# mcdiarmid/waveforms

Measured on AMD Instinct MI355X. Metric: SOQPSK-TG Msym/s mod+Viterbi-detect @8sps, higher is better.
Workload: dtype f64; 1 GPU; SOQPSK-TG 1e+07 symbols @8 sps, modulate + AWGN + PT matched filter + 4-state Viterbi detect (BASELINE configs[1]); waveform=soqpsk, sps=8, prbs=PN23, noise=Philox4x32-10 + Box-Muller (device), fuse=175, streams=1, detector_warmup_rows=16, detector_form=lanes (one chunk per lane), parallelism=independent trial blocks x1

## Files before the change

waveforms_amd/csrc/wf_common.h:

```cpp
#pragma once
#include <hip/hip_runtime.h>
#include <stdint.h>

#include <atomic>
#include <map>
#include <mutex>
#include <vector>
#include <string>

#include "../../include/wfhip.h"

#define WF_WAVE 64

void wf_set_error(const char *fmt, ...);

#define WF_HIP(call)                                                                     \
    do {                                                                                 \
        hipError_t e_ = (call);                                                          \
        if (e_ != hipSuccess) {                                                          \
            wf_set_error("%s failed: %s (%s:%d)", #call, hipGetErrorString(e_), __FILE__, \
                         __LINE__);                                                      \
            return WF_ERR_HIP;                                                           \
        }                                                                                \
    } while (0)

#define WF_REQUIRE(cond, ...)          \
    do {                               \
        if (!(cond)) {                 \
            wf_set_error(__VA_ARGS__); \
            return WF_ERR_VALUE;       \
        }                              \
    } while (0)

#define WF_LAUNCH_CHECK() WF_HIP(hipGetLastError())

enum { WF_FAULT_SCAN_TIMEOUT = 1u, WF_FAULT_LIVE_TABLE = 2u };

struct wf_lfsr_tables {
    uint64_t host[64][64];
    uint64_t *dev = nullptr;
    uint64_t f_even = 0, f_odd = 0, f_m2 = 0, f_m1 = 0;
    bool f_ready = false;
};

struct wf_ctx {
    int device = 0;
    int cus = 256;
    int64_t opt[WF_OPT_COUNT] = {0};
    uint64_t *d_scan = nullptr;
    size_t scan_words = 0;
    unsigned *d_fault = nullptr;
    unsigned *h_fault = nullptr;
    uint8_t *d_tables = nullptr;
    uint8_t h_tables_cache[2048] = {0};
    int tables_cached = 0;
    hipEvent_t tables_event = nullptr;
    hipStream_t tables_stream = nullptr;
    bool tables_pending = false;
    uint64_t *d_fsm_scratch = nullptr;
    size_t fsm_scratch_words = 0;
    int *h_small = nullptr;
    int *d_small = nullptr;
    std::map<uint64_t, wf_lfsr_tables *> lfsr;
    double *d_mod_scratch = nullptr;
    size_t mod_scratch_words = 0;
    double *d_vit_edge = nullptr;
    size_t vit_edge_words = 0;
    unsigned long long *d_vit_unmerged = nullptr;
    hipEvent_t *events = nullptr;
    void *pipe_stream = nullptr;
    void *pipe_stream2 = nullptr;
    void *pipe_pro = nullptr, *pipe_main = nullptr;
    hipEvent_t pipe_pro_done = nullptr;
    hipEvent_t pipe_back_go = nullptr;
    bool pipe_back_go_valid = false;
    bool pipe_front_recorded = false;
    bool pipe_front_on_main = false;
    hipEvent_t pipe_front = nullptr, pipe_done[2] = {nullptr, nullptr};
    bool pipe_done_valid[2] = {false, false};
    int pipe_set = 0;
    std::map<uint64_t, uint32_t> promises;
    std::mutex promises_lock;
    double *h_iter = nullptr;
    double *d_iter = nullptr;
    void *h_mailbox = nullptr;
    void *d_mailbox = nullptr;
    void *iter_stream = nullptr;
    const void *iter_last_state = nullptr;
    std::atomic_flag iter_lock = ATOMIC_FLAG_INIT;
    bool iter_closing = false;
};

static inline hipStream_t wf_stream(void *s) { return reinterpret_cast<hipStream_t>(s); }

int wf_ctx_reserve_scan(wf_ctx *ctx, size_t words);
int wf_ctx_reserve_fsm(wf_ctx *ctx, size_t words);
int wf_ctx_reserve_mod(wf_ctx *ctx, size_t words);
int wf_iter_server_stop(wf_ctx *ctx);
int wf_ctx_reserve_vit(wf_ctx *ctx, size_t words);

struct lfsr_emit_args;
int wf_lfsr_generate_dyn(wf_ctx *ctx, int degree, uint64_t mask, uint64_t state, uint64_t skip,
                         const uint64_t *d_dyn_skip, uint8_t *d_bits, int64_t n, uint64_t *h_state_out, void *stream,
                         const struct lfsr_emit_args *emit = nullptr);
int wf_lfsr_generate_map(wf_ctx *ctx, int degree, uint64_t mask, uint64_t state, uint64_t skip, uint8_t *d_bits, int64_t nbits,
                         int map_kind, int8_t *d_symbols, void *stream);
int wf_soqpsk_prbs_encode(wf_ctx *ctx, int degree, uint64_t mask, uint64_t state, uint64_t skip, const uint8_t *h_next,
                          const int8_t *h_out, uint8_t *d_bits, int64_t n, int8_t *d_symbols, void *stream, void *mid_event = nullptr);
int wf_awgn_mf_bank_dyn(wf_ctx *ctx, const double *d_signal_ri, int64_t nsamp, double rot_re, double rot_im,
                        double sigma, uint64_t seed, uint64_t stream_id, uint64_t first_index,
                        const uint64_t *d_dyn_index, const double *d_taps_ri, int nfilt, int ntaps, int64_t first,
                        int step, int64_t ncols, double *d_out_ri, void *stream, int pack_par0 = -1);
int wf_viterbi4_detect_packed(wf_ctx *ctx, const double *d_rows4, int64_t ncalls, int differential, int warmup,
                              uint8_t *d_bits, int8_t *d_syms, double *d_state, void *stream);
int wf_cpm_modulate_window(wf_ctx *ctx, const int8_t *d_symbols, int64_t sym_origin, int64_t nloc, int64_t nsym_total,
                           const double *d_h, int nh, const double *d_pulse, int ntaps, int sps, double phi0,
                           int64_t tile_lo, int64_t ntiles, double *d_out_ri, int64_t out_origin,
                           const uint64_t *d_q_in, uint64_t *d_q_out, int64_t q_out_tile, void *stream);
struct wf_mcb_opts {
    const double *pam_factor = nullptr;
    bool cpm_paired = false;
    int runs_hint = 0;
    int scratch_slot = -1;
};
int wf_mod_chan_bank_packed(wf_ctx *ctx, const int8_t *d_symbols, int64_t nsym, const double *d_h, int nh,
                            const double *d_pulse, int ntaps, int sps, double phi0, const double *d_mf_taps, double rot_re,
                            double rot_im, double sigma, uint64_t seed, uint64_t stream_id, uint64_t first_index,
                            int64_t first, int64_t ncols, int pack_par0, double *d_rows4, void *stream, int mf_ntaps = 0,
                            const wf_mcb_opts *opts = nullptr, int stage = 3);
int wf_mod_chan_bank_window(wf_ctx *ctx, const int8_t *d_symbols, int64_t sym_origin, int64_t nloc, int64_t nsym_total,
                            const double *d_h, int nh, const double *d_pulse, int ntaps, int sps, double phi0,
                            int64_t tile_lo, int64_t ntiles, const uint64_t *d_q_in, uint64_t *d_q_out, int64_t q_out_tile,
                            const double *d_mf_taps, double rot_re, double rot_im, double sigma, uint64_t seed,
                            uint64_t stream_id, uint64_t first_index, const uint64_t *d_dyn_index, int64_t first,
                            int64_t k_lo, int64_t ncols, int pack_par0, double *d_rows4, void *stream, int cpm_nf = 0, int cpm_nh = 1,
                            int stage = 3, int mf_ntaps = 0, const wf_mcb_opts *opts = nullptr);
int wf_mod_chan_bank_applies(int64_t nsym, int nh, int ntaps, int sps, int mf_ntaps, int64_t first);
int wf_link_join_internal(wf_ctx *ctx, void *stream);
int wf_mod_chan_cpm_rows_applies(int64_t nsym, int nh, int ntaps, int sps, int nfilt, int ntm, int64_t start0);
int wf_mod_chan_cpm_rows(wf_ctx *ctx, const int8_t *d_symbols, int64_t nsym, const double *d_h, int nh, const double *d_pulse,
                         int ntaps, int sps, double phi0, const double *d_templates, int nfilt, int ntm, int64_t start0,
                         double rot_re, double rot_im, double sigma, uint64_t seed, uint64_t stream_id, int64_t ncalls,
                         double *d_rows, void *stream, const wf_mcb_opts *opts = nullptr);
int wf_mod_chan_samples_applies(int64_t nsym, int nh, int ntaps, int sps);
int wf_mod_chan_samples(wf_ctx *ctx, const int8_t *d_symbols, int64_t nsym, const double *d_h, int nh, const double *d_pulse, int ntaps,
                        int sps, double phi0, double rot_re, double rot_im, double sigma, uint64_t seed, uint64_t stream_id,
                        uint64_t first_index, double *d_out_ri, void *stream);
int wf_mod_chan_samples_window(wf_ctx *ctx, const int8_t *d_symbols, int64_t sym_origin, int64_t nloc, int64_t nsym_total, const double *d_h, int nh,
                               const double *d_pulse, int ntaps, int sps, double phi0, int64_t tile_lo, int64_t ntiles, const uint64_t *d_q_in,
                               uint64_t *d_q_out, int64_t q_out_tile, double rot_re, double rot_im, double sigma, uint64_t seed, uint64_t stream_id,
                               uint64_t first_index, double *d_out_ri, int64_t out_origin, int64_t out_hi, void *stream);
int wf_promise_verified(wf_ctx *ctx, int kind, const void *const *d_ptrs, const size_t *nbytes, int nptrs, void *stream,
                        bool (*check)(const unsigned char *const *host, const size_t *nbytes, const void *arg), const void *arg, const char *what);
int wf_fsm_encode_core(wf_ctx *ctx, const uint8_t *h_next, const int8_t *h_out, int columns, int states, int card,
                       const uint8_t *d_bits, int64_t nbits, int64_t i0, int state0, const int *d_state_in,
                       int8_t *d_symbols, int *h_state_out, int *d_state_at, int64_t at_index, void *stream);

static inline int wf_grid_for(int64_t work_items, int per_block, int max_blocks)
{
    int64_t b = (work_items + per_block - 1) / per_block;
// ... 374 lines not shown
```

waveforms_amd/csrc/wf_cpm_detect.hip:

```cpp
#include <stddef.h>
#include <stdlib.h>
#include <string.h>

#include <type_traits>

#include "wf_cpm_detect.h"
#include "wf_link.h"

#define CPM_THREADS 256
#define CPM_WAVES (CPM_THREADS / WF_WAVE)
#define CPM_GROUPS 4
#define CPM_TB 4
#define CPM_DEFAULT_WARMUP 256
#define CPM_XS 68

struct cpm_tables {
    uint8_t dest[3][16][4];
    uint16_t info[3][16][4];
};

struct cpm_vit_params {
    int M, lgM, p, nh, K0, K1, Lp, NC, D, S, NF;
    int CH, W;
    int64_t ncalls, nchunks;
// ... 1052 lines not shown
extern "C" int wf_cpm_link_run(wf_ctx *ctx, const wf_cpm_link_config *cfg, void *d_workspace, int64_t workspace_bytes,
                               int64_t *d_counts, int64_t *h_compared, void *stream)
{
    WF_REQUIRE(ctx && cfg && d_workspace && d_counts, "wf_cpm_link_run: NULL argument");
    cpm_link_layout L;
    WF_REQUIRE(cpm_make_layout(cfg, L), "wf_cpm_link_run: bad configuration");
    WF_REQUIRE((reinterpret_cast<uintptr_t>(d_workspace) & 255) == 0, "wf_cpm_link_run: workspace must be 256-byte aligned");
    WF_REQUIRE((int64_t)L.total <= workspace_bytes, "wf_cpm_link_run: workspace too small (%lld < %lld)",
               (long long)workspace_bytes, (long long)L.total);
    WF_REQUIRE(cfg->d_h && cfg->d_pulse && cfg->d_templates && cfg->d_rot_cs, "wf_cpm_link_run: NULL table pointer");
    char *w = static_cast<char *>(d_workspace);
    const bool piped = (cfg->fuse & 32) != 0 && L.ncalls > 0 && !cpm_link_samples_form_quad(cfg, L);
    int rc;
    if (piped) {
        const int64_t set_bytes = round_up((int64_t)L.total, 256);
        if ((rc = link_pipe_open(ctx, "wf_cpm_link_run", set_bytes, workspace_bytes, true)) || (rc = link_pipe_select(ctx, set_bytes, w, stream))) return rc;
    } else if ((rc = wf_link_join_internal(ctx, stream))) {
        return rc;
    }
    uint8_t *bits = reinterpret_cast<uint8_t *>(w + L.off_bits);
    int8_t *syms = reinterpret_cast<int8_t *>(w + L.off_syms);
    double *sig = reinterpret_cast<double *>(w + L.off_sig);
    double *rows = reinterpret_cast<double *>(w + L.off_rows);
    uint8_t *dec = reinterpret_cast<uint8_t *>(w + L.off_dec);
    hipEvent_t *ev;
    if ((rc = link_stage_events(ctx, "wf_cpm_link_run", cfg->event_slot, ev))) return rc;
    if ((rc = mark(ev, 0, stream))) return rc;
    rc = (cfg->fuse & 16) ? 1 : wf_lfsr_generate_map(ctx, cfg->degree, cfg->mask, cfg->state, cfg->skip, bits, L.nbits, cfg->mapper_kind, syms, stream);
    if (rc < 0) return rc;
    if (rc == 1) {
        if ((rc = wf_lfsr_generate(ctx, cfg->degree, cfg->mask, cfg->state, cfg->skip, bits, L.nbits, nullptr, stream))) return rc;
        if ((rc = mark(ev, 1, stream))) return rc;
        if ((rc = wf_symbol_map(ctx, cfg->mapper_kind, bits, L.nbits, 0, 0, 0, syms, stream))) return rc;
    } else {
        if ((rc = mark(ev, 1, stream))) return rc;
    }
    if ((rc = mark(ev, 2, stream))) return rc;
    bool fused_all = false, samples_form = false;
    const bool samples_quad = cpm_link_samples_form_quad(cfg, L);
    if (cpm_link_samples_form(ctx, cfg, L)) {
        if (!samples_quad && (rc = cpm_check_paired(ctx, cfg, L.nfilt, L.ntm, stream))) return rc;
        rc = wf_mod_chan_samples(ctx, syms, cfg->nsym, cfg->d_h, cfg->det.nh, cfg->d_pulse, cfg->ntaps, cfg->sps, M_PI / 4, cos(-M_PI / 4), sin(-M_PI / 4),
                                 cfg->sigma, cfg->seed, cfg->stream_id, 0, sig, stream);
        if (rc < 0) return rc;
        samples_form = fused_all = rc == 0;
    }
    if (!fused_all && (cfg->fuse & 8) && (cfg->fuse & 2) && L.ncalls > 0) {
        wf_mcb_opts mo;
        mo.runs_hint = piped ? (L.nfilt == 4 ? 16 : 8) : 0;
        mo.cpm_paired = (cfg->fuse & 64) != 0;
        if (mo.cpm_paired && (rc = cpm_check_paired(ctx, cfg, L.nfilt, L.ntm, stream))) return rc;
        rc = wf_mod_chan_cpm_rows(ctx, syms, cfg->nsym, cfg->d_h, cfg->det.nh, cfg->d_pulse, cfg->ntaps, cfg->sps, M_PI / 4, cfg->d_templates,
                                  L.nfilt, L.ntm, L.start0, cos(-M_PI / 4), sin(-M_PI / 4), cfg->sigma, cfg->seed, cfg->stream_id, L.ncalls,
                                  rows, stream, &mo);
        if (rc < 0) return rc;
        fused_all = rc == 0;
    }
    if (!fused_all) {
        rc = wf_cpm_modulate_c128(ctx, syms, cfg->nsym, cfg->d_h, cfg->det.nh, cfg->d_pulse, cfg->ntaps, cfg->sps, M_PI / 4, sig, stream);
        if (rc < 0) return rc;
        WF_REQUIRE(rc == 0, "wf_cpm_link_run: burst / pulse outside the fused modulator (%lld symbols, %d taps)",
                   (long long)cfg->nsym, cfg->ntaps);
    }
    if ((rc = mark(ev, 3, stream)) || (rc = mark(ev, 4, stream))) return rc;
    if (fused_all) {
        if ((rc = mark(ev, 5, stream))) return rc;
    } else if (cfg->fuse & 2) {
        if ((rc = mark(ev, 5, stream))) return rc;
        if ((rc = wf_cpm_awgn_mf_rows_c128(ctx, sig, L.npts, cos(-M_PI / 4), sin(-M_PI / 4), cfg->sigma, cfg->seed, cfg->stream_id, 0,
                                           cfg->d_templates, cfg->det.nh, L.nfilt, L.ntm, L.start0, cfg->sps, L.ncalls, rows, stream))) return rc;
    } else {
        if ((rc = wf_awgn_c128(ctx, sig, L.npts, cos(-M_PI / 4), sin(-M_PI / 4), cfg->sigma, cfg->seed, cfg->stream_id, 0, sig, stream))) return rc;
        if ((rc = mark(ev, 5, stream))) return rc;
        if ((rc = wf_cpm_mf_rows_c128(ctx, sig, L.npts, cfg->d_templates, cfg->det.nh, L.nfilt, L.ntm, L.start0, cfg->sps, L.ncalls,
                                      rows, stream))) return rc;
    }
    void *back = stream;
    const bool two_back = piped && !wf_cpm_quad_applies(&cfg->det) && !wf_cpm_wide_applies(&cfg->det);
    const int edge_slot = two_back ? ctx->pipe_set : -1;
    if (piped) {
        back = two_back && ctx->pipe_set ? ctx->pipe_stream2 : ctx->pipe_stream;
        WF_HIP(hipEventRecord(ctx->pipe_front, wf_stream(stream)));
        WF_HIP(hipStreamWaitEvent(wf_stream(back), ctx->pipe_front, 0));
    }
    if ((rc = mark(ev, 6, back))) return rc;
    if (samples_form && samples_quad) {
        const cpm_mf_source mf{cfg->d_templates, L.npts, 0, L.start0};
        if ((rc = wf_cpm_viterbi_detect_in(ctx, &cfg->det, cfg->d_rot_cs, sig, L.ncalls, cfg->warmup, dec, nullptr, back, 0, 0, piped, &mf, -1))) return rc;
    } else if (samples_form) {
        const cpm_mf_source mf{cfg->d_templates, L.npts - L.start0, 0};
        if ((rc = wf_cpm_viterbi_detect_in(ctx, &cfg->det, cfg->d_rot_cs, sig + 2 * L.start0, L.ncalls, cfg->warmup, dec, nullptr, back,
                                           (int64_t)L.off_sig + 16 * L.start0, (int64_t)(L.total - L.off_sig) - L.npts * 16, piped, &mf, edge_slot)))
            return rc;
    } else if ((rc = wf_cpm_viterbi_detect_in(ctx, &cfg->det, cfg->d_rot_cs, rows, L.ncalls, cfg->warmup, dec, nullptr, back, (int64_t)L.off_rows,
                                              (int64_t)(L.total - L.off_rows) - L.ncalls * L.nfilt * 16, piped, nullptr, edge_slot)))
        return rc;
    if ((rc = mark(ev, 7, back))) return rc;
    const int64_t skip = cfg->skip_head > 0 ? cfg->skip_head : 0;
    int64_t m = L.ncalls - cfg->det.D + 1 - skip;
    if (m < 0) m = 0;
    if (m > 0)
        if ((rc = wf_cpm_count_errors(ctx, dec + skip + cfg->det.D - 1, syms + skip, cfg->det.M, m, d_counts, back))) return rc;
    if ((rc = mark(ev, 8, back))) return rc;
    if (piped && (rc = link_pipe_close(ctx, back))) return rc;
    if (h_compared) *h_compared = m;
    return WF_OK;
}

struct cpm_stream_layout : link_chunk_window {
    int64_t N, B, tile_len, spt, ntiles_total, halo, ncalls_total, m_total;
    size_t off_bits, off_syms, off_rows, off_dec, total;
    cpm_link_layout L;
    bool ok;
};

static cpm_stream_layout cpm_make_stream_layout(const wf_cpm_link_config *cfg, int64_t B, int64_t c)
{
    cpm_stream_layout S{};
    if (!cpm_make_layout(cfg, S.L) || B <= 0 || c < 0) return S;
    S.N = cfg->nsym; S.B = B;
    S.ok = wf_mod_tile_geometry(cfg->sps, cfg->ntaps, cfg->nsym, &S.tile_len, &S.spt, &S.ntiles_total) == 0;
    if (!S.ok || S.spt <= 0) { S.ok = false; return S; }
    S.halo = round_up(S.spt + 48 + cfg->det.D, 16);
    S.ncalls_total = S.L.ncalls;
    const int64_t skip = cfg->skip_head > 0 ? cfg->skip_head : 0;
    S.m_total = S.ncalls_total - cfg->det.D + 1 - skip;
    if (S.m_total < 0) S.m_total = 0;
    S.ok = B % S.spt == 0 && B % 128 == 0 && B >= 4 * S.halo &&
           ((cfg->fuse & 8) && (cfg->fuse & 2) &&
            wf_mod_chan_cpm_rows_applies(cfg->nsym, cfg->det.nh, cfg->ntaps, cfg->sps, S.L.nfilt, S.L.ntm, S.L.start0));
    static_cast<link_chunk_window &>(S) = link_chunk_window_of(B, c, S.halo, S.N, S.ncalls_total, S.spt, S.ntiles_total);
    size_t o = 0;
    const int64_t win = B + 2 * S.halo + 32;
    S.off_bits = o; o += (size_t)round_up(win * S.L.bps, 256);
    S.off_syms = o; o += (size_t)round_up(win, 256);
    S.off_rows = o; o += (size_t)round_up(B * S.L.nfilt * 16, 256);
    S.off_dec = o;  o += (size_t)round_up(B + 16, 256);
    S.total = o;
    return S;
}

extern "C" int64_t wf_cpm_link_stream_workspace_bytes(const wf_cpm_link_config *cfg, int64_t chunk_symbols)
{
    const cpm_stream_layout S = cpm_make_stream_layout(cfg, chunk_symbols, 0);
    return S.ok ? (int64_t)S.total : -1;
}

extern "C" int wf_cpm_link_stream_layout(const wf_cpm_link_config *cfg, int64_t chunk_symbols, int64_t chunk_index, int64_t *info8)
{
    if (!info8) return WF_ERR_VALUE;
    const cpm_stream_layout S = cpm_make_stream_layout(cfg, chunk_symbols, chunk_index);
    if (!S.ok) return WF_ERR_VALUE;
    info8[0] = S.ncols; info8[1] = S.k_lo; info8[2] = (int64_t)S.off_dec; info8[3] = (int64_t)S.off_syms;
    info8[4] = S.ws; info8[5] = S.ncalls_total; info8[6] = S.spt; info8[7] = (int64_t)S.off_rows;
    return WF_OK;
}

extern "C" int wf_cpm_link_stream_chunk(wf_ctx *ctx, const wf_cpm_link_config *cfg, int64_t chunk_symbols, int64_t chunk_index,
                                        void *d_state, void *d_workspace, int64_t workspace_bytes, int64_t *d_counts,
                                        int64_t *h_compared, void *stream)
{
    return wf_cpm_link_stream_chunk_phase(ctx, cfg, chunk_symbols, chunk_index, d_state, d_workspace, workspace_bytes, d_counts, h_compared, 7, stream);
}

extern "C" int wf_cpm_link_stream_chunk_phase(wf_ctx *ctx, const wf_cpm_link_config *cfg, int64_t chunk_symbols, int64_t chunk_index,
                                              void *d_state, void *d_workspace, int64_t workspace_bytes, int64_t *d_counts,
// ... 74 lines not shown
```

waveforms_amd/csrc/wf_ctx.hip:

```cpp
#include <stdarg.h>
#include <stdio.h>

#include "wf_common.h"

static thread_local char g_err[512] = "";

void wf_set_error(const char *fmt, ...)
{
    va_list ap;
    va_start(ap, fmt);
    vsnprintf(g_err, sizeof(g_err), fmt, ap);
    va_end(ap);
}

extern "C" const char *wf_version(void) { return "waveforms-amd 0.1.0 (gfx950)"; }
extern "C" const char *wf_last_error_string(void) { return g_err; }

extern "C" int wf_ctx_create(int device, wf_ctx **out)
{
    WF_REQUIRE(out != nullptr, "wf_ctx_create: out is NULL");
    int ndev = 0;
    WF_HIP(hipGetDeviceCount(&ndev));
    WF_REQUIRE(device >= 0 && device < ndev, "wf_ctx_create: device %d of %d", device, ndev);
    WF_HIP(hipSetDevice(device));
    wf_ctx *c = new wf_ctx();
    c->device = device;
    (void)hipDeviceGetAttribute(&c->cus, hipDeviceAttributeMultiprocessorCount, device);
    if (c->cus < 1) c->cus = 256;
    c->opt[WF_OPT_PIPE_RESERVE_CUS] = -1;
    WF_HIP(hipMalloc(&c->d_fault, 64));
    WF_HIP(hipMemset(c->d_fault, 0, 64));
    WF_HIP(hipHostMalloc(&c->h_fault, 64, hipHostMallocDefault));
    WF_HIP(hipMalloc(&c->d_tables, 4096));
    WF_HIP(hipMalloc(&c->d_vit_unmerged, 4 * sizeof(unsigned long long)));
    WF_HIP(hipMemset(c->d_vit_unmerged, 0, 4 * sizeof(unsigned long long)));
    WF_HIP(hipMalloc(&c->d_small, 256));
    WF_HIP(hipHostMalloc(&c->h_small, 256, hipHostMallocDefault));
    *out = c;
    int rc = wf_ctx_reserve_scan(c, 1 << 16);
    if (rc) return rc;
    return wf_ctx_reserve_fsm(c, 1 << 16);
}

extern "C" int wf_ctx_destroy(wf_ctx *c)
{
    if (!c) return WF_OK;
    (void)hipSetDevice(c->device);
    (void)wf_iter_server_stop(c);
    (void)hipDeviceSynchronize();
    for (auto &kv : c->lfsr) {
        if (kv.second->dev) (void)hipFree(kv.second->dev);
        delete kv.second;
    }
    if (c->events) {
        for (int k = 0; k < WF_LINK_EVENT_SLOTS * (WF_LINK_STAGES + 1); ++k) (void)hipEventDestroy(c->events[k]);
        delete[] c->events;
    }
    if (c->pipe_front) (void)hipEventDestroy(c->pipe_front);
    for (int k = 0; k < 2; ++k)
        if (c->pipe_done[k]) (void)hipEventDestroy(c->pipe_done[k]);
    if (c->pipe_stream) (void)hipStreamDestroy(static_cast<hipStream_t>(c->pipe_stream));
    if (c->pipe_stream2) (void)hipStreamDestroy(static_cast<hipStream_t>(c->pipe_stream2));
    if (c->pipe_pro) (void)hipStreamDestroy(static_cast<hipStream_t>(c->pipe_pro));
    if (c->pipe_main) (void)hipStreamDestroy(static_cast<hipStream_t>(c->pipe_main));
    if (c->pipe_pro_done) (void)hipEventDestroy(c->pipe_pro_done);
    if (c->pipe_back_go) (void)hipEventDestroy(c->pipe_back_go);
    if (c->d_scan) (void)hipFree(c->d_scan);
    if (c->d_fsm_scratch) (void)hipFree(c->d_fsm_scratch);
    if (c->d_mod_scratch) (void)hipFree(c->d_mod_scratch);
    if (c->d_vit_edge) (void)hipFree(c->d_vit_edge);
    if (c->d_vit_unmerged) (void)hipFree(c->d_vit_unmerged);
    if (c->d_fault) (void)hipFree(c->d_fault);
    if (c->h_fault) (void)hipHostFree(c->h_fault);
    if (c->d_tables) (void)hipFree(c->d_tables);
    if (c->tables_event) (void)hipEventDestroy(c->tables_event);
    if (c->d_small) (void)hipFree(c->d_small);
    if (c->h_small) (void)hipHostFree(c->h_small);
    if (c->h_iter) (void)hipHostFree(c->h_iter);
    if (c->iter_stream) (void)hipStreamDestroy(static_cast<hipStream_t>(c->iter_stream));
    if (c->h_mailbox) (void)hipHostFree(c->h_mailbox);
    delete c;
    return WF_OK;
}

extern "C" int wf_ctx_retire(wf_ctx *c)
{
    if (!c) return WF_OK;
    (void)hipSetDevice(c->device);
    (void)wf_iter_server_stop(c);
    if (c->pipe_stream) (void)hipStreamSynchronize(static_cast<hipStream_t>(c->pipe_stream));
    if (c->pipe_stream2) (void)hipStreamSynchronize(static_cast<hipStream_t>(c->pipe_stream2));
    if (c->pipe_pro) (void)hipStreamSynchronize(static_cast<hipStream_t>(c->pipe_pro));
    if (c->pipe_main) (void)hipStreamSynchronize(static_cast<hipStream_t>(c->pipe_main));
    return WF_OK;
}

int wf_link_join_internal(wf_ctx *c, void *stream)
{
    if (!c) return WF_OK;
    for (int k = 0; k < 2; ++k)
        if (c->pipe_done_valid[k]) WF_HIP(hipStreamWaitEvent(wf_stream(stream), c->pipe_done[k], 0));
    return WF_OK;
}

extern "C" int wf_link_join(wf_ctx *c, void *stream)
{
    WF_REQUIRE(c != nullptr, "wf_link_join: ctx is NULL");
    return wf_link_join_internal(c, stream);
}

extern "C" int wf_ctx_set_option(wf_ctx *c, int key, int64_t value)
{
    WF_REQUIRE(c != nullptr, "wf_ctx_set_option: ctx is NULL");
    WF_REQUIRE(key >= 0 && key < WF_OPT_COUNT, "wf_ctx_set_option: unknown option %d", key);
    bool ok = true;
    switch (key) {
    case WF_OPT_CPM_FORM: ok = value >= 0 && value <= 2; break;
    case WF_OPT_CPM_CHUNK_CALLS: ok = value >= 0 && value <= 8192; break;
    case WF_OPT_DET_REPAIR: case WF_OPT_DET_FINAL_VERIFY: case WF_OPT_ITERATION_SERVER: ok = value == 0 || value == 1; break;
    case WF_OPT_MCB_TAIL_PERMILLE: ok = value >= -1 && value <= 16000; break;
    case WF_OPT_PIPE_RESERVE_CUS: ok = value >= -1 && value <= 128; break;
    case WF_OPT_CPM_SAMPLES_MIN_CALLS: ok = value == 0 || (value >= 4096 && value <= ((int64_t)1 << 40)); break;
    case WF_OPT_SOFT_CHUNK_CALLS: ok = value >= 0 && value <= 8192; break;
    case WF_OPT_CPM_SOFT_CHUNK_CALLS: ok = value >= 0 && value <= 8192; break;
    }
    WF_REQUIRE(ok, "wf_ctx_set_option: value %lld outside the range of option %d", (long long)value, key);
    c->opt[key] = value;
    return WF_OK;
}

extern "C" int wf_ctx_get_option(wf_ctx *c, int key, int64_t *value)
{
    WF_REQUIRE(c != nullptr && value != nullptr, "wf_ctx_get_option: NULL argument");
    WF_REQUIRE(key >= 0 && key < WF_OPT_COUNT, "wf_ctx_get_option: unknown option %d", key);
    *value = c->opt[key];
    return WF_OK;
}

extern "C" int wf_ctx_check(wf_ctx *c, void *stream)
{
    WF_REQUIRE(c != nullptr, "wf_ctx_check: ctx is NULL");
    {
        const int rj = wf_link_join_internal(c, stream);
        if (rj) return rj;
    }
    WF_HIP(hipMemcpyAsync(c->h_fault, c->d_fault, sizeof(unsigned), hipMemcpyDeviceToHost,
                          wf_stream(stream)));
    WF_HIP(hipStreamSynchronize(wf_stream(stream)));
    unsigned f = *c->h_fault;
    if (f) {
        WF_HIP(hipMemsetAsync(c->d_fault, 0, sizeof(unsigned), wf_stream(stream)));
        wf_set_error("device fault word 0x%x (bit0 = scan hand-off timeout, bit1 = malformed live-window table)", f);
        return WF_ERR_DEVICE;
    }
    return WF_OK;
}

int wf_promise_verified(wf_ctx *c, int kind, const void *const *d_ptrs, const size_t *nbytes, int nptrs, void *stream,
                        bool (*check)(const unsigned char *const *host, const size_t *nbytes, const void *arg), const void *arg, const char *what)
{
    uint64_t key = 1469598103934665603ull;
    auto mix = [&](uint64_t v) {
        for (int b = 0; b < 8; ++b) {
            key ^= (v >> (8 * b)) & 0xFFull;
            key *= 1099511628211ull;
        }
    };
    mix((uint64_t)kind);
    for (int i = 0; i < nptrs; ++i) {
        WF_REQUIRE(d_ptrs[i] != nullptr && nbytes[i] > 0 && nbytes[i] <= (1u << 16), "%s: operand %d is NULL or larger than 64 KB", what, i);
        mix((uint64_t)reinterpret_cast<uintptr_t>(d_ptrs[i]));
        mix((uint64_t)nbytes[i]);
    }
    std::lock_guard<std::mutex> guard(c->promises_lock);
    auto it = c->promises.find(key);
    if (it != c->promises.end()) {
// ... 86 lines not shown
```

waveforms_amd/csrc/wf_link.h:

```cpp
#pragma once
#include "wf_common.h"

static inline int64_t round_up(int64_t v, int64_t a) { return (v + a - 1) / a * a; }

static inline int link_pipe_open(wf_ctx *ctx, const char *fn, int64_t set_bytes, int64_t workspace_bytes, bool second)
{
    WF_REQUIRE(2 * set_bytes <= workspace_bytes, "%s: fuse bit 5 needs two sets of intermediates (%lld bytes)", fn, (long long)(2 * set_bytes));
    WF_HIP(hipSetDevice(ctx->device));
    hipStream_t ps;
    if (!ctx->pipe_stream) {
        WF_HIP(hipStreamCreateWithFlags(&ps, hipStreamNonBlocking));
        ctx->pipe_stream = ps;
        WF_HIP(hipEventCreateWithFlags(&ctx->pipe_front, hipEventDisableTiming));
        for (int k = 0; k < 2; ++k) WF_HIP(hipEventCreateWithFlags(&ctx->pipe_done[k], hipEventDisableTiming));
    }
    if (second && !ctx->pipe_stream2) {
        WF_HIP(hipStreamCreateWithFlags(&ps, hipStreamNonBlocking));
        ctx->pipe_stream2 = ps;
    }
    return WF_OK;
}

static inline int link_pipe_select(wf_ctx *ctx, int64_t set_bytes, char *&w, void *waiter, bool on_main = false)
{
    if (ctx->pipe_front_on_main != on_main && ctx->pipe_front_recorded) WF_HIP(hipStreamWaitEvent(wf_stream(waiter), ctx->pipe_front, 0));
    ctx->pipe_front_on_main = on_main;
    ctx->pipe_front_recorded = true;
    w += (int64_t)ctx->pipe_set * set_bytes;
    if (ctx->pipe_done_valid[ctx->pipe_set]) WF_HIP(hipStreamWaitEvent(wf_stream(waiter), ctx->pipe_done[ctx->pipe_set], 0));
    return WF_OK;
}

static inline int link_pipe_close(wf_ctx *ctx, void *back)
{
    WF_HIP(hipEventRecord(ctx->pipe_done[ctx->pipe_set], wf_stream(back)));
    ctx->pipe_done_valid[ctx->pipe_set] = true;
    ctx->pipe_set ^= 1;
    return WF_OK;
}

static inline int link_stage_events(wf_ctx *ctx, const char *fn, int event_slot, hipEvent_t *&ev)
{
    ev = nullptr;
    if (event_slot < 0) return WF_OK;
    WF_REQUIRE(event_slot < WF_LINK_EVENT_SLOTS, "%s: event_slot %d", fn, event_slot);
    if (!ctx->events) {
        ctx->events = new hipEvent_t[WF_LINK_EVENT_SLOTS * (WF_LINK_STAGES + 1)];
        for (int k = 0; k < WF_LINK_EVENT_SLOTS * (WF_LINK_STAGES + 1); ++k) WF_HIP(hipEventCreate(&ctx->events[k]));
    }
    ev = ctx->events + event_slot * (WF_LINK_STAGES + 1);
    return WF_OK;
}

static inline int mark(hipEvent_t *ev, int k, void *stream)
{
    if (ev) WF_HIP(hipEventRecord(ev[k], wf_stream(stream)));
    return WF_OK;
}

struct link_chunk_window {
    int64_t k_lo, ncols, ws, nloc, tile_lo, tile_hi, ntiles, q_out_tile;
};

static inline link_chunk_window link_chunk_window_of(int64_t B, int64_t c, int64_t halo, int64_t N, int64_t ncalls_total, int64_t spt, int64_t ntiles_total)
{
    link_chunk_window W;
    W.k_lo = c * B;
    const int64_t k_hi = W.k_lo + B < ncalls_total ? W.k_lo + B : ncalls_total;
    W.ncols = k_hi > W.k_lo ? k_hi - W.k_lo : 0;
    W.ws = c * B - halo > 0 ? c * B - halo : 0;
    const int64_t we = (c + 1) * B + halo < N ? (c + 1) * B + halo : N;
    W.nloc = we > W.ws ? we - W.ws : 0;
    W.tile_lo = spt > 0 && c * B / spt - 1 > 0 ? c * B / spt - 1 : 0;
    W.tile_hi = spt > 0 ? (c + 1) * B / spt + 1 : 0;
    if (W.tile_hi > ntiles_total) W.tile_hi = ntiles_total;
    W.ntiles = W.tile_hi > W.tile_lo ? W.tile_hi - W.tile_lo : 0;
    const int64_t next_tile_lo = spt > 0 ? (c + 1) * B / spt - 1 : 0;
    W.q_out_tile = (next_tile_lo >= W.tile_lo && next_tile_lo < W.tile_hi) ? next_tile_lo - W.tile_lo : -1;
    return W;
}

struct soqpsk_trellis_tables {
    uint8_t next[2][4][2];
    int8_t outp[2][4][2];
};

static inline soqpsk_trellis_tables soqpsk_trellis(int differential)
{
    static const int8_t kOut[2][8] = {{0, 2, 0, -2, -2, 0, 2, 0}, {0, -2, 2, 0, 0, 2, -2, 0}};
    soqpsk_trellis_tables T;
    for (int c = 0; c < 2; ++c)
        for (int b = 0; b < 8; ++b) {
            const int s = b >> 1, flip = differential ? (c == 0 ? (s >> 1) : (s & 1)) : 0, inp = (b & 1) ^ flip;
            T.next[c][s][inp] = (uint8_t)(c == 0 ? (s & 1) + 2 * (b & 1) : (s & 2) + (b & 1));
            T.outp[c][s][inp] = kOut[c][b];
        }
    return T;
}
```

waveforms_amd/csrc/wf_pipeline.hip:

```cpp
#include "wf_link.h"

__global__ void time_axis_kernel(int64_t n, double step, double *__restrict__ out)
{
    const int64_t stride = (int64_t)gridDim.x * blockDim.x;
    for (int64_t k = (int64_t)blockIdx.x * blockDim.x + threadIdx.x; k < n; k += stride)
        out[k] = (double)k * step;
}

extern "C" int wf_time_axis_f64(wf_ctx *ctx, int64_t n, double step, double *d_out, void *stream)
{
    WF_REQUIRE(ctx && n >= 0, "wf_time_axis_f64: bad argument");
    if (n == 0) return WF_OK;
    WF_REQUIRE(d_out != nullptr, "wf_time_axis_f64: NULL output");
    WF_HIP(hipSetDevice(ctx->device));
    hipLaunchKernelGGL(time_axis_kernel, dim3(wf_grid_for(n, 256, 4096)), dim3(256), 0, wf_stream(stream), n,
                       step, d_out);
    WF_LAUNCH_CHECK();
    return WF_OK;
}

struct link_layout {
    int64_t nsym, npts, ncols, first;
    size_t off_bits, off_syms, off_freq, off_sig, off_mf, off_dbits, off_dsyms, total;
};
// ... 23 lines not shown
static int link_warmup(const wf_link_config *cfg) { return cfg->warmup; }

static bool link_packed_rows8(const wf_link_config *cfg)
{
    return (cfg->fuse & 4) && (cfg->fuse & 2) && cfg->sps == 8 && cfg->mf_nfilt == 3;
}

static bool link_one_kernel(const wf_link_config *cfg)
{
    if ((cfg->fuse & 15) != 15 || cfg->mf_nfilt != 3 || cfg->sps < 2) return false;
    int64_t first = (-(int64_t)cfg->timing_offset) % cfg->sps;
    if (first < 0) first += cfg->sps;
    return wf_mod_chan_bank_applies(cfg->nsym, 1, cfg->ntaps, cfg->sps, cfg->mf_ntaps, first) != 0;
}

static bool link_packed_rows(const wf_link_config *cfg) { return link_packed_rows8(cfg) || link_one_kernel(cfg); }

static bool link_pipelined(const wf_link_config *cfg) { return (cfg->fuse & 32) && link_one_kernel(cfg); }

static bool link_factor_matches(const unsigned char *const *host, const size_t *, const void *arg)
{
    const int nt = *static_cast<const int *>(arg);
    const double *taps = reinterpret_cast<const double *>(host[0]);
    const double *b = reinterpret_cast<const double *>(host[1]);
    const double *G = b + 2 * nt;
    double big = 0.0, worst = 0.0;
    for (int s = 0; s < 3; ++s)
        for (int t = 0; t < nt; ++t) {
            const double re = G[4 * s] * b[t] + G[4 * s + 2] * b[nt + t], im = G[4 * s + 1] * b[t] + G[4 * s + 3] * b[nt + t];
            const double tr = taps[2 * (s * nt + t)], ti = taps[2 * (s * nt + t) + 1];
            const double d = hypot(re - tr, im - ti), m = hypot(tr, ti);
            if (!(d == d)) return false;
            if (d > worst) worst = d;
            if (m > big) big = m;
        }
    return worst <= 1e-12 * big;
}
static int link_check_factor(wf_ctx *ctx, const wf_link_config *cfg, void *stream)
{
    if (!cfg->d_mf_factor || cfg->mf_ntaps == cfg->sps + 1 || cfg->mf_nfilt != 3 || cfg->mf_ntaps < 1) return WF_OK;
    const int nt = cfg->mf_ntaps;
    const void *ptrs[2] = {cfg->d_mf_taps, cfg->d_mf_factor};
    const size_t nb[2] = {(size_t)3 * nt * 16, (size_t)(2 * nt + 12) * 8};
    return wf_promise_verified(ctx, 2, ptrs, nb, 2, stream, link_factor_matches, &nt,
                               "wf_link_config.d_mf_factor does not reproduce d_mf_taps (taps[s] != sum_k G[s][k] b_k to 1e-12)");
}

extern "C" int64_t wf_link_workspace_bytes(const wf_link_config *cfg)
{
    if (!cfg || cfg->nsym < 1 || cfg->sps < 1) return -1;
    const int64_t one = (int64_t)make_layout(cfg->nsym, cfg->sps, cfg->ntaps, cfg->mf_nfilt, 2, cfg->timing_offset).total;
    return link_pipelined(cfg) ? 2 * round_up(one, 256) : one;
}

static hipStream_t link_masked_stream(const wf_ctx *ctx, int reserve)
{
    hipStream_t s = nullptr;
    if (reserve > 0 && reserve < ctx->cus) {
        const int words = (ctx->cus + 31) / 32;
        std::vector<uint32_t> mask((size_t)words, 0u);
        for (int cu = reserve; cu < ctx->cus; ++cu) mask[(size_t)(cu / 32)] |= 1u << (cu % 32);
        if (hipExtStreamCreateWithCUMask(&s, (uint32_t)words, mask.data()) == hipSuccess) return s;
        (void)hipGetLastError();
        s = nullptr;
    }
    if (hipStreamCreateWithFlags(&s, hipStreamDefault) != hipSuccess) return nullptr;
    return s;
}

extern "C" int wf_link_run(wf_ctx *ctx, const wf_link_config *cfg, void *d_workspace, int64_t workspace_bytes,
                           int64_t *d_counts, int64_t *h_compared, void *stream)
{
    WF_REQUIRE(ctx && cfg && d_workspace && d_counts, "wf_link_run: NULL argument");
    WF_REQUIRE(cfg->nsym >= 1 && cfg->sps >= 1 && cfg->mf_nfilt == 3, "wf_link_run: bad configuration");
    WF_REQUIRE((reinterpret_cast<uintptr_t>(d_workspace) & 255) == 0, "wf_link_run: workspace must be 256-byte aligned");
    const int length = 2;
    const link_layout L = make_layout(cfg->nsym, cfg->sps, cfg->ntaps, cfg->mf_nfilt, length, cfg->timing_offset);
    WF_REQUIRE((int64_t)L.total <= workspace_bytes, "wf_link_run: workspace too small (%lld < %lld)",
               (long long)workspace_bytes, (long long)L.total);
    WF_REQUIRE(L.npts >= cfg->mf_ntaps, "wf_link_run: burst shorter than the matched filter");
    char *w = static_cast<char *>(d_workspace);
    const bool piped = link_pipelined(cfg) && L.ncols > 0;
    void *s_pro = stream, *s_main = stream;
    bool ahead = false;
    int slot = -1, rc;
    if (piped) {
        const int64_t set_bytes = round_up((int64_t)L.total, 256);
        if ((rc = link_pipe_open(ctx, "wf_link_run", set_bytes, workspace_bytes, false))) return rc;
        const int64_t rsv = ctx->opt[WF_OPT_PIPE_RESERVE_CUS];
        ahead = rsv > 0 || (rsv < 0 && cfg->mf_ntaps == cfg->sps + 1);
        if (ahead) {
            if (!ctx->pipe_pro) {
                hipStream_t sp;
                WF_HIP(hipStreamCreateWithFlags(&sp, hipStreamDefault));
                ctx->pipe_pro = sp;
            }
            if (!ctx->pipe_main) {
                ctx->pipe_main = link_masked_stream(ctx, rsv < 0 ? 0 : (int)rsv);
                WF_REQUIRE(ctx->pipe_main != nullptr, "wf_link_run: could not create the front end's stream");
            }
            if (!ctx->pipe_pro_done) WF_HIP(hipEventCreateWithFlags(&ctx->pipe_pro_done, hipEventDisableTiming));
            if (!ctx->pipe_back_go) WF_HIP(hipEventCreateWithFlags(&ctx->pipe_back_go, hipEventDisableTiming));
            s_pro = stream ? stream : ctx->pipe_pro;
            s_main = ctx->pipe_main;
            slot = ctx->pipe_set;
        }
        if ((rc = link_pipe_select(ctx, set_bytes, w, s_pro, ahead))) return rc;
    } else if ((rc = wf_link_join_internal(ctx, stream))) {
        return rc;
    }
    uint8_t *bits = reinterpret_cast<uint8_t *>(w + L.off_bits);
    int8_t *syms = reinterpret_cast<int8_t *>(w + L.off_syms);
    double *freq = reinterpret_cast<double *>(w + L.off_freq);
    double *sig = reinterpret_cast<double *>(w + L.off_sig);
    double *mf = reinterpret_cast<double *>(w + L.off_mf);
    uint8_t *dbits = reinterpret_cast<uint8_t *>(w + L.off_dbits);
    int8_t *dsyms = reinterpret_cast<int8_t *>(w + L.off_dsyms);

    const soqpsk_trellis_tables T = soqpsk_trellis(cfg->differential);
    hipEvent_t *ev;
    if ((rc = link_stage_events(ctx, "wf_link_run", cfg->event_slot, ev))) return rc;
    if ((rc = mark(ev, 0, s_pro))) return rc;
    rc = (cfg->fuse & 16) ? 1 : wf_soqpsk_prbs_encode(ctx, cfg->degree, cfg->mask, cfg->state, cfg->skip, &T.next[0][0][0], &T.outp[0][0][0], bits,
                                                       cfg->nsym, syms, s_pro, ev ? (void *)ev[1] : nullptr);
    if (rc < 0) return rc;
    if (rc == 1) {
        if ((rc = wf_lfsr_generate(ctx, cfg->degree, cfg->mask, cfg->state, cfg->skip, bits, cfg->nsym, nullptr, s_pro))) return rc;
        if ((rc = mark(ev, 1, s_pro))) return rc;
        if ((rc = wf_fsm_encode(ctx, &T.next[0][0][0], &T.outp[0][0][0], 2, 4, 1, bits, cfg->nsym, 0, 0, syms, nullptr, s_pro))) return rc;
    }
    if (!ahead && (rc = mark(ev, 2, s_pro))) return rc;
    bool fused_all = false;
    if (link_one_kernel(cfg) && L.ncols > 0) {
        wf_mcb_opts mo;
        mo.pam_factor = cfg->d_mf_factor;
        mo.scratch_slot = slot;
        if ((rc = link_check_factor(ctx, cfg, stream))) return rc;
        for (int stage = ahead ? 1 : 3; stage <= (ahead ? 2 : 3); ++stage) {
            if (ahead && stage == 2) {
                if ((rc = mark(ev, 2, s_pro))) return rc;
                WF_HIP(hipEventRecord(ctx->pipe_pro_done, wf_stream(s_pro)));
                WF_HIP(hipStreamWaitEvent(wf_stream(s_main), ctx->pipe_pro_done, 0));
                if (ctx->pipe_back_go_valid) WF_HIP(hipStreamWaitEvent(wf_stream(s_main), ctx->pipe_back_go, 0));
                if ((rc = mark(ev, 3, s_main))) return rc;
            }
            rc = wf_mod_chan_bank_packed(ctx, syms, cfg->nsym, cfg->d_h, 1, cfg->d_pulse, cfg->ntaps, cfg->sps, M_PI / 4, cfg->d_mf_taps,
                                         cos(-M_PI / 4), sin(-M_PI / 4), cfg->sigma, cfg->seed, cfg->stream_id, 0, L.first, L.ncols, 0,
                                         mf, stage == 1 ? s_pro : s_main, cfg->mf_ntaps, &mo, stage);
            if (rc < 0) return rc;
            WF_REQUIRE(rc == 0, "wf_link_run: internal: the one-kernel front end refused a configuration wf_mod_chan_bank_applies accepted");
        }
        fused_all = true;
    }
    if (fused_all) {
        if (!ahead && (rc = mark(ev, 3, s_main))) return rc;
        if ((rc = mark(ev, 4, s_main)) || (rc = mark(ev, 5, s_main))) return rc;
        void *back = stream;
        if (piped) {
            back = ctx->pipe_stream;
            WF_HIP(hipEventRecord(ctx->pipe_front, wf_stream(s_main)));
            WF_HIP(hipStreamWaitEvent(wf_stream(back), ctx->pipe_front, 0));
            if (ahead) {
                WF_HIP(hipEventRecord(ctx->pipe_back_go, wf_stream(back)));
                ctx->pipe_back_go_valid = true;
            }
        }
        if ((rc = mark(ev, 6, back))) return rc;
        rc = wf_viterbi4_detect_packed(ctx, mf, L.ncols, cfg->differential, link_warmup(cfg), dbits, dsyms, nullptr, back);
        if (rc) return rc;
        if ((rc = mark(ev, 7, back))) return rc;
        int64_t m_ = L.ncols - length;
        if (m_ > cfg->nsym) m_ = cfg->nsym;
        if (m_ < 0) m_ = 0;
        if ((rc = wf_count_errors(ctx, dsyms + length, syms, dbits + length, bits, m_, d_counts, back))) return rc;
        if ((rc = mark(ev, 8, back))) return rc;
        if (piped && (rc = link_pipe_close(ctx, back))) return rc;
        if (h_compared) *h_compared = m_;
        return WF_OK;
    }
    bool fused_mod = false;
    if (cfg->fuse & 1) {
        rc = wf_cpm_modulate_c128(ctx, syms, cfg->nsym, cfg->d_h, 1, cfg->d_pulse, cfg->ntaps, cfg->sps, M_PI / 4, sig, stream);
        if (rc < 0) return rc;
        fused_mod = rc == 0;
    }
    if (fused_mod) {
        if ((rc = mark(ev, 3, stream))) return rc;
    } else {
        if ((rc = wf_upsample_fir_f64(ctx, syms, cfg->nsym, cfg->d_h, 1, cfg->d_pulse, cfg->ntaps, cfg->sps, freq, stream))) return rc;
        if ((rc = mark(ev, 3, stream))) return rc;
        if ((rc = wf_phase_cexp_f64(ctx, freq, L.npts, cfg->sps, M_PI / 4, 0.0, sig, nullptr, stream))) return rc;
    }
    if ((rc = mark(ev, 4, stream))) return rc;
    const double rot_re = cos(-M_PI / 4), rot_im = sin(-M_PI / 4);
    const bool fused_chan = (cfg->fuse & 2) && L.ncols > 0;
    if (!fused_chan)
        if ((rc = wf_awgn_c128(ctx, sig, L.npts, rot_re, rot_im, cfg->sigma, cfg->seed, cfg->stream_id, 0, sig, stream))) return rc;
    if ((rc = mark(ev, 5, stream))) return rc;
    int64_t m = L.ncols - length;
    if (m > cfg->nsym) m = cfg->nsym;
    if (m < 0) m = 0;
    const bool packed = fused_chan && link_packed_rows8(cfg);
    if (L.ncols > 0) {
        if (packed)
            rc = wf_awgn_mf_bank_dyn(ctx, sig, L.npts, rot_re, rot_im, cfg->sigma, cfg->seed, cfg->stream_id, 0, nullptr,
                                     cfg->d_mf_taps, cfg->mf_nfilt, cfg->mf_ntaps, L.first, cfg->sps, L.ncols, mf, stream, 0);
        else if (fused_chan)
            rc = wf_awgn_mf_bank_c128(ctx, sig, L.npts, rot_re, rot_im, cfg->sigma, cfg->seed, cfg->stream_id, 0,
                                      cfg->d_mf_taps, cfg->mf_nfilt, cfg->mf_ntaps, L.first, cfg->sps, L.ncols, mf, stream);
        else
            rc = wf_mf_bank_c128(ctx, sig, L.npts, cfg->d_mf_taps, cfg->mf_nfilt, cfg->mf_ntaps, L.first, cfg->sps,
                                 L.ncols, mf, stream);
        if (rc) return rc;
        if ((rc = mark(ev, 6, stream))) return rc;
        if (packed)
            rc = wf_viterbi4_detect_packed(ctx, mf, L.ncols, cfg->differential, link_warmup(cfg), dbits, dsyms, nullptr, stream);
        else
            rc = wf_viterbi4_detect(ctx, mf, L.ncols, cfg->differential, link_warmup(cfg), dbits, dsyms, nullptr, stream);
        if (rc) return rc;
    } else {
        if ((rc = mark(ev, 6, stream))) return rc;
    }
    if ((rc = mark(ev, 7, stream))) return rc;
    if (m > 0)
        if ((rc = wf_count_errors(ctx, dsyms + length, syms, dbits + length, bits, m, d_counts, stream))) return rc;
    if ((rc = mark(ev, 8, stream))) return rc;
    if (h_compared) *h_compared = m;
    return WF_OK;
}

extern "C" int wf_link_stage_ms(wf_ctx *ctx, int event_slot, float *h_ms)
{
    WF_REQUIRE(ctx && h_ms && event_slot >= 0 && event_slot < WF_LINK_EVENT_SLOTS && ctx->events,
               "wf_link_stage_ms: no events recorded in slot %d", event_slot);
    hipEvent_t *ev = ctx->events + event_slot * (WF_LINK_STAGES + 1);
    WF_HIP(hipEventSynchronize(ev[WF_LINK_STAGES]));
    for (int k = 0; k < WF_LINK_STAGES; ++k) WF_HIP(hipEventElapsedTime(&h_ms[k], ev[k], ev[k + 1]));
    return WF_OK;
}

extern "C" int wf_link_layout(const wf_link_config *cfg, int64_t *info8)
{
    if (!cfg || !info8 || cfg->nsym < 1 || cfg->sps < 1) return WF_ERR_VALUE;
    const link_layout L = make_layout(cfg->nsym, cfg->sps, cfg->ntaps, cfg->mf_nfilt, 2, cfg->timing_offset);
    info8[0] = L.ncols; info8[2] = (int64_t)L.off_dbits; info8[3] = (int64_t)L.off_dsyms;
    info8[4] = (int64_t)L.off_sig; info8[6] = L.npts; info8[7] = (int64_t)L.off_mf;
    info8[1] = link_one_kernel(cfg) ? 1 : 0;
    info8[5] = link_packed_rows(cfg) ? 32 : 16 * cfg->mf_nfilt;
// ... 221 lines not shown
```

Measured before the change: 23070 Msym/s.

## Chain each pipelined call onto one of two alternating streams at 8 sps

For the ahead-pipelined 8 sps configuration, each call now runs prologue, front end and Viterbi back end on one of two alternating streams instead of splitting them across separate prologue, main and back streams. Ordering between consecutive calls is kept with front and done events, and a new back-order helper makes a back end wait for the previous set's completion when streams switch. The aim is to drop cross-stream event handoffs within a call while still letting consecutive calls overlap. The risk is lost overlap between stages of one call and added complexity in the event dependencies.

After: 23450 Msym/s (median of 6 runs). +1.6%, better.

```diff
diff --git a/waveforms_amd/csrc/wf_common.h b/waveforms_amd/csrc/wf_common.h
--- a/waveforms_amd/csrc/wf_common.h
+++ b/waveforms_amd/csrc/wf_common.h
@@ -74,8 +74,14 @@
     hipEvent_t pipe_pro_done = nullptr;
     hipEvent_t pipe_back_go = nullptr;
     bool pipe_back_go_valid = false;
+    void *pipe_chain[2] = {nullptr, nullptr};
+    hipEvent_t pipe_call = nullptr;
+    hipEvent_t pipe_chain_pro = nullptr;
+    bool pipe_chain_pro_valid = false;
+    void *pipe_back_last = nullptr;
     bool pipe_front_recorded = false;
-    bool pipe_front_on_main = false;
+    int pipe_front_kind = 0;
+    uint64_t pipe_carries = 0;
     hipEvent_t pipe_front = nullptr, pipe_done[2] = {nullptr, nullptr};
     bool pipe_done_valid[2] = {false, false};
     int pipe_set = 0;
diff --git a/waveforms_amd/csrc/wf_cpm_detect.hip b/waveforms_amd/csrc/wf_cpm_detect.hip
--- a/waveforms_amd/csrc/wf_cpm_detect.hip
+++ b/waveforms_amd/csrc/wf_cpm_detect.hip
@@ -1158,6 +1158,7 @@
         back = two_back && ctx->pipe_set ? ctx->pipe_stream2 : ctx->pipe_stream;
         WF_HIP(hipEventRecord(ctx->pipe_front, wf_stream(stream)));
         WF_HIP(hipStreamWaitEvent(wf_stream(back), ctx->pipe_front, 0));
+        if ((rc = link_pipe_back_order(ctx, back))) return rc;
     }
     if ((rc = mark(ev, 6, back))) return rc;
     if (samples_form && samples_quad) {
diff --git a/waveforms_amd/csrc/wf_ctx.hip b/waveforms_amd/csrc/wf_ctx.hip
--- a/waveforms_amd/csrc/wf_ctx.hip
+++ b/waveforms_amd/csrc/wf_ctx.hip
@@ -65,6 +65,10 @@
     if (c->pipe_main) (void)hipStreamDestroy(static_cast<hipStream_t>(c->pipe_main));
     if (c->pipe_pro_done) (void)hipEventDestroy(c->pipe_pro_done);
     if (c->pipe_back_go) (void)hipEventDestroy(c->pipe_back_go);
+    for (int k = 0; k < 2; ++k)
+        if (c->pipe_chain[k]) (void)hipStreamDestroy(static_cast<hipStream_t>(c->pipe_chain[k]));
+    if (c->pipe_call) (void)hipEventDestroy(c->pipe_call);
+    if (c->pipe_chain_pro) (void)hipEventDestroy(c->pipe_chain_pro);
     if (c->d_scan) (void)hipFree(c->d_scan);
     if (c->d_fsm_scratch) (void)hipFree(c->d_fsm_scratch);
     if (c->d_mod_scratch) (void)hipFree(c->d_mod_scratch);
@@ -92,6 +96,8 @@
     if (c->pipe_stream2) (void)hipStreamSynchronize(static_cast<hipStream_t>(c->pipe_stream2));
     if (c->pipe_pro) (void)hipStreamSynchronize(static_cast<hipStream_t>(c->pipe_pro));
     if (c->pipe_main) (void)hipStreamSynchronize(static_cast<hipStream_t>(c->pipe_main));
+    for (int k = 0; k < 2; ++k)
+        if (c->pipe_chain[k]) (void)hipStreamSynchronize(static_cast<hipStream_t>(c->pipe_chain[k]));
     return WF_OK;
 }
 
diff --git a/waveforms_amd/csrc/wf_link.h b/waveforms_amd/csrc/wf_link.h
--- a/waveforms_amd/csrc/wf_link.h
+++ b/waveforms_amd/csrc/wf_link.h
@@ -3,16 +3,17 @@
 
 static inline int64_t round_up(int64_t v, int64_t a) { return (v + a - 1) / a * a; }
 
-static inline int link_pipe_open(wf_ctx *ctx, const char *fn, int64_t set_bytes, int64_t workspace_bytes, bool second)
+static inline int link_pipe_open(wf_ctx *ctx, const char *fn, int64_t set_bytes, int64_t workspace_bytes, bool second, bool side = true)
 {
     WF_REQUIRE(2 * set_bytes <= workspace_bytes, "%s: fuse bit 5 needs two sets of intermediates (%lld bytes)", fn, (long long)(2 * set_bytes));
     WF_HIP(hipSetDevice(ctx->device));
     hipStream_t ps;
-    if (!ctx->pipe_stream) {
+    if (!ctx->pipe_front) WF_HIP(hipEventCreateWithFlags(&ctx->pipe_front, hipEventDisableTiming));
+    for (int k = 0; k < 2; ++k)
+        if (!ctx->pipe_done[k]) WF_HIP(hipEventCreateWithFlags(&ctx->pipe_done[k], hipEventDisableTiming));
+    if (side && !ctx->pipe_stream) {
         WF_HIP(hipStreamCreateWithFlags(&ps, hipStreamNonBlocking));
         ctx->pipe_stream = ps;
-        WF_HIP(hipEventCreateWithFlags(&ctx->pipe_front, hipEventDisableTiming));
-        for (int k = 0; k < 2; ++k) WF_HIP(hipEventCreateWithFlags(&ctx->pipe_done[k], hipEventDisableTiming));
     }
     if (second && !ctx->pipe_stream2) {
         WF_HIP(hipStreamCreateWithFlags(&ps, hipStreamNonBlocking));
@@ -21,13 +22,24 @@
     return WF_OK;
 }
 
-static inline int link_pipe_select(wf_ctx *ctx, int64_t set_bytes, char *&w, void *waiter, bool on_main = false)
+static inline int link_pipe_select(wf_ctx *ctx, int64_t set_bytes, char *&w, void *waiter, int kind = 0, uint64_t carries = 0)
 {
-    if (ctx->pipe_front_on_main != on_main && ctx->pipe_front_recorded) WF_HIP(hipStreamWaitEvent(wf_stream(waiter), ctx->pipe_front, 0));
-    ctx->pipe_front_on_main = on_main;
+    if ((ctx->pipe_front_kind != kind || ctx->pipe_carries != carries) && ctx->pipe_front_recorded)
+        WF_HIP(hipStreamWaitEvent(wf_stream(waiter), ctx->pipe_front, 0));
+    ctx->pipe_front_kind = kind;
+    ctx->pipe_carries = carries;
     ctx->pipe_front_recorded = true;
     w += (int64_t)ctx->pipe_set * set_bytes;
     if (ctx->pipe_done_valid[ctx->pipe_set]) WF_HIP(hipStreamWaitEvent(wf_stream(waiter), ctx->pipe_done[ctx->pipe_set], 0));
+    return WF_OK;
+}
+
+static inline int link_pipe_back_order(wf_ctx *ctx, void *back)
+{
+    const void *last = ctx->pipe_back_last;
+    const bool chains = back == ctx->pipe_chain[0] || back == ctx->pipe_chain[1] || last == ctx->pipe_chain[0] || last == ctx->pipe_chain[1];
+    if (last && last != back && chains && ctx->pipe_done_valid[ctx->pipe_set ^ 1])
+        WF_HIP(hipStreamWaitEvent(wf_stream(back), ctx->pipe_done[ctx->pipe_set ^ 1], 0));
     return WF_OK;
 }
 
@@ -35,6 +47,7 @@
 {
     WF_HIP(hipEventRecord(ctx->pipe_done[ctx->pipe_set], wf_stream(back)));
     ctx->pipe_done_valid[ctx->pipe_set] = true;
+    ctx->pipe_back_last = back;
     ctx->pipe_set ^= 1;
     return WF_OK;
 }
diff --git a/waveforms_amd/csrc/wf_pipeline.hip b/waveforms_amd/csrc/wf_pipeline.hip
--- a/waveforms_amd/csrc/wf_pipeline.hip
+++ b/waveforms_amd/csrc/wf_pipeline.hip
@@ -129,14 +129,28 @@
     char *w = static_cast<char *>(d_workspace);
     const bool piped = link_pipelined(cfg) && L.ncols > 0;
     void *s_pro = stream, *s_main = stream;
-    bool ahead = false;
+    bool ahead = false, chain = false, had_front = false;
     int slot = -1, rc;
     if (piped) {
         const int64_t set_bytes = round_up((int64_t)L.total, 256);
-        if ((rc = link_pipe_open(ctx, "wf_link_run", set_bytes, workspace_bytes, false))) return rc;
         const int64_t rsv = ctx->opt[WF_OPT_PIPE_RESERVE_CUS];
         ahead = rsv > 0 || (rsv < 0 && cfg->mf_ntaps == cfg->sps + 1);
-        if (ahead) {
+        chain = ahead && rsv < 0 && cfg->sps == 8;
+        if ((rc = link_pipe_open(ctx, "wf_link_run", set_bytes, workspace_bytes, false, !chain))) return rc;
+        if (chain) {
+            for (int s = 0; s < 2; ++s)
+                if (!ctx->pipe_chain[s]) {
+                    hipStream_t sc;
+                    WF_HIP(hipStreamCreateWithFlags(&sc, hipStreamNonBlocking));
+                    ctx->pipe_chain[s] = sc;
+                }
+            if (!ctx->pipe_call) WF_HIP(hipEventCreateWithFlags(&ctx->pipe_call, hipEventDisableTiming));
+            if (!ctx->pipe_chain_pro) WF_HIP(hipEventCreateWithFlags(&ctx->pipe_chain_pro, hipEventDisableTiming));
+            s_pro = s_main = ctx->pipe_chain[ctx->pipe_set];
+            slot = ctx->pipe_set;
+            WF_HIP(hipEventRecord(ctx->pipe_call, wf_stream(stream)));
+            WF_HIP(hipStreamWaitEvent(wf_stream(s_pro), ctx->pipe_call, 0));
+        } else if (ahead) {
             if (!ctx->pipe_pro) {
                 hipStream_t sp;
                 WF_HIP(hipStreamCreateWithFlags(&sp, hipStreamDefault));
@@ -152,7 +166,9 @@
             s_main = ctx->pipe_main;
             slot = ctx->pipe_set;
         }
-        if ((rc = link_pipe_select(ctx, set_bytes, w, s_pro, ahead))) return rc;
+        had_front = ctx->pipe_front_recorded;
+        const uint64_t carries = ahead ? ((uint64_t)cfg->nsym << 20) | ((uint64_t)cfg->sps << 10) | (uint64_t)cfg->ntaps : 0;
+        if ((rc = link_pipe_select(ctx, set_bytes, w, s_pro, chain ? 2 : (ahead ? 1 : 0), carries))) return rc;
     } else if ((rc = wf_link_join_internal(ctx, stream))) {
         return rc;
     }
@@ -171,7 +187,9 @@
     rc = (cfg->fuse & 16) ? 1 : wf_soqpsk_prbs_encode(ctx, cfg->degree, cfg->mask, cfg->state, cfg->skip, &T.next[0][0][0], &T.outp[0][0][0], bits,
                                                        cfg->nsym, syms, s_pro, ev ? (void *)ev[1] : nullptr);
     if (rc < 0) return rc;
-    if (rc == 1) {
+    const bool generic = rc == 1;
+    if (generic) {
+        if (chain && ctx->pipe_chain_pro_valid) WF_HIP(hipStreamWaitEvent(wf_stream(s_pro), ctx->pipe_chain_pro, 0));
         if ((rc = wf_lfsr_generate(ctx, cfg->degree, cfg->mask, cfg->state, cfg->skip, bits, cfg->nsym, nullptr, s_pro))) return rc;
         if ((rc = mark(ev, 1, s_pro))) return rc;
         if ((rc = wf_fsm_encode(ctx, &T.next[0][0][0], &T.outp[0][0][0], 2, 4, 1, bits, cfg->nsym, 0, 0, syms, nullptr, s_pro))) return rc;
@@ -186,9 +204,17 @@
         for (int stage = ahead ? 1 : 3; stage <= (ahead ? 2 : 3); ++stage) {
             if (ahead && stage == 2) {
                 if ((rc = mark(ev, 2, s_pro))) return rc;
-                WF_HIP(hipEventRecord(ctx->pipe_pro_done, wf_stream(s_pro)));
-                WF_HIP(hipStreamWaitEvent(wf_stream(s_main), ctx->pipe_pro_done, 0));
-                if (ctx->pipe_back_go_valid) WF_HIP(hipStreamWaitEvent(wf_stream(s_main), ctx->pipe_back_go, 0));
+                if (chain) {
+                    if (generic) {
+                        WF_HIP(hipEventRecord(ctx->pipe_chain_pro, wf_stream(s_pro)));
+                        ctx->pipe_chain_pro_valid = true;
+                    }
+                    if (had_front) WF_HIP(hipStreamWaitEvent(wf_stream(s_main), ctx->pipe_front, 0));
+                } else {
+                    WF_HIP(hipEventRecord(ctx->pipe_pro_done, wf_stream(s_pro)));
+                    WF_HIP(hipStreamWaitEvent(wf_stream(s_main), ctx->pipe_pro_done, 0));
+                    if (ctx->pipe_back_go_valid) WF_HIP(hipStreamWaitEvent(wf_stream(s_main), ctx->pipe_back_go, 0));
+                }
                 if ((rc = mark(ev, 3, s_main))) return rc;
             }
             rc = wf_mod_chan_bank_packed(ctx, syms, cfg->nsym, cfg->d_h, 1, cfg->d_pulse, cfg->ntaps, cfg->sps, M_PI / 4, cfg->d_mf_taps,
@@ -204,13 +230,14 @@
         if ((rc = mark(ev, 4, s_main)) || (rc = mark(ev, 5, s_main))) return rc;
         void *back = stream;
         if (piped) {
-            back = ctx->pipe_stream;
+            back = chain ? s_main : ctx->pipe_stream;
             WF_HIP(hipEventRecord(ctx->pipe_front, wf_stream(s_main)));
-            WF_HIP(hipStreamWaitEvent(wf_stream(back), ctx->pipe_front, 0));
-            if (ahead) {
+            if (!chain) WF_HIP(hipStreamWaitEvent(wf_stream(back), ctx->pipe_front, 0));
+            if (ahead && !chain) {
                 WF_HIP(hipEventRecord(ctx->pipe_back_go, wf_stream(back)));
                 ctx->pipe_back_go_valid = true;
             }
+            if ((rc = link_pipe_back_order(ctx, back))) return rc;
         }
         if ((rc = mark(ev, 6, back))) return rc;
         rc = wf_viterbi4_detect_packed(ctx, mf, L.ncols, cfg->differential, link_warmup(cfg), dbits, dsyms, nullptr, back);
```
